# ShunyaoWang/quadruped_locomotion

Hardware: AMD Instinct MI355X
Metric: control-step QP solves/sec (18-DoF, 4-contact) at 1/2/4/8 MI355X (higher is better)
Workload: dtype f64

## Files before the change

### quadruped_locomotion_amd/csrc/force_qp_coop.hpp

```cpp
#pragma once

#include "coop_lanes.hpp"

#if defined(__FAST_MATH__) || (defined(__FINITE_MATH_ONLY__) && __FINITE_MATH_ONLY__)
#error "force_qp_coop.hpp needs IEEE inf / NaN semantics: do not build this translation unit with -ffast-math / -ffinite-math-only"
#endif

#ifndef QL_QP_BLOCK_STAMP
#define QL_QP_BLOCK_STAMP(slot) QL_BLOCK_STAMP(slot)
#endif
namespace qlamd {
namespace coop {

constexpr int kCoopLdsDoubles = 12 * 12;
constexpr int kMaxRefinePasses = 8;
#ifndef QLAMD_REFINE_AGAIN
#define QLAMD_REFINE_AGAIN 1e-3
#endif
constexpr double kRefineAgain = QLAMD_REFINE_AGAIN;
constexpr int kDropSlot = 48, kZeroSlot = 60, kWarmSlot = 61;
constexpr int kForceQpNrmRows = 5, kForceQpNrmRowsTorque = 8;
template <class T>
constexpr T one_v = T(1);
constexpr int kStatusWarmRejected = 6;
struct ForceQp {
  double Gm[12];
  double g0;
  double nb[3], t1[3], t2[3];
  double myn, myt1, myt2;
  double mu, f_min;
  bool on, comp;
  int nS;
  int refine_passes;
  double jrow[3], jcol[3];
  double tq_up, tq_lo;
  unsigned long long warm;
  unsigned stance;
  bool build_set;
};

__device__ __forceinline__ void force_qp_objective(const double S[6], double w_reg, double foot, unsigned stance, bool row_on,
                                                   const double F[6], const double *jrow, double w_tau_jt0, double Gm[12],
                                                   double &g0, double w_tau = 0.0) {
  const int lr = threadIdx.x & 15, leg = lr >> 2, c = lr & 3;
  const int myidx = 3 * leg + c;
  double r[4][3];
  static_for<12>([&](auto J) { constexpr int j = J; r[j / 3][j % 3] = bcv<j>(foot); });
  const double rl[3] = {quad_bc<0>(foot), quad_bc<1>(foot), quad_bc<2>(foot)};
  const double a[3] = {sel(c == 1, -rl[2], sel(c == 2, rl[1], 0.0)), sel(c == 0, rl[2], sel(c == 2, -rl[0], 0.0)),
                       sel(c == 0, -rl[1], sel(c == 1, rl[0], 0.0))};
  const double sa[3] = {S[3] * a[0], S[4] * a[1], S[5] * a[2]};
  const double Sfc = pick3(S, c);
#pragma unroll
  for (int m = 0; m < 4; m++) {
    const bool both = row_on && ((stance >> m) & 1u);
    const double xp = r[m][0], yp = r[m][1], zp = r[m][2];
    const double e0 = sa[1] * zp - sa[2] * yp;
    const double e1 = -sa[0] * zp + sa[2] * xp;
    const double e2 = sa[0] * yp - sa[1] * xp;
    Gm[3 * m + 0] = both ? e0 + (c == 0 ? Sfc : 0.0) : 0.0;
    Gm[3 * m + 1] = both ? e1 + (c == 1 ? Sfc : 0.0) : 0.0;
    Gm[3 * m + 2] = both ? e2 + (c == 2 ? Sfc : 0.0) : 0.0;
  }
  if (jrow) {
    double jj[3];
    static_for<3>([&](auto Bq) {
      constexpr int bq = Bq;
      jj[bq] = jrow[0] * quad_bc<bq>(jrow[0]) + jrow[1] * quad_bc<bq>(jrow[1]) + jrow[2] * quad_bc<bq>(jrow[2]);
    });
#pragma unroll
    for (int m = 0; m < 4; m++) {
      const bool own = row_on && m == leg;
#pragma unroll
      for (int bq = 0; bq < 3; bq++) Gm[3 * m + bq] += own ? w_tau * jj[bq] : 0.0;
    }
  }
#pragma unroll
  for (int j = 0; j < 12; j++)
    if (c < 3 && j == myidx) Gm[j] += row_on ? w_reg : 1.0;
  const double Fc = pick3(F, c);
  const double ST[3] = {S[3] * F[3], S[4] * F[4], S[5] * F[5]};
  const double g0v = -(Sfc * Fc + (a[0] * ST[0] + a[1] * ST[1] + a[2] * ST[2]) + w_tau_jt0);
  g0 = sel(row_on, g0v, 0.0);
}

template <bool kTorque, bool kWarm = false, int kLegs = 4, bool kRounds = true>
__device__ __forceinline__ int force_qp_coop(const ForceQp &Q, double *lds_row, double *lds_nrm, double &x, int &iters_out,
                                             unsigned long long *ws_out = nullptr) {
  using mask_t = std::conditional_t<kTorque, unsigned long long, unsigned>;
  constexpr int kKinds = kTorque ? 11 : 5;
  static_assert(kLegs == 2 || kLegs == 4, "legs in front of the row");
  constexpr int kV = 3 * kLegs;
  const int lr = threadIdx.x & 15, leg = lr >> 2, c = lr & 3;
  const bool comp = Q.comp && leg < kLegs, on = Q.on, row_on = comp && on;
  const int myidx = 3 * leg + c, nS = Q.nS;
  const double eps = 2.220446049250313e-16;
  const double inf = INFINITY;
  const double mu = Q.mu, f_min = Q.f_min, g0 = Q.g0;
  const double myn = Q.myn, myt1 = Q.myt1, myt2 = Q.myt2;
  const double *nb = Q.nb, *t1 = Q.t1, *t2 = Q.t2, *Gm = Q.Gm;
  double H[kV];
  double c1 = 0.0, c2 = 0.0;
  {
#pragma unroll
    for (int j = 0; j < kV; j++) H[j] = Gm[j];
    {
      double diag = 0.0;
#pragma unroll
      for (int j = 0; j < kV; j++) diag = (j == myidx) ? Gm[j] : diag;
      c1 = row_sum(sel(row_on, diag, 0.0));
    }
    bool bad = false;
    double my_pivot = 1.0;
    double d = bcv<0>(H[0]);
    static_for<kV>([&](auto K) {
      constexpr int k = K;
      bad = bad || !(d > 0.0);
      const double p = rcp_nr1(d);
      const bool piv = comp && (myidx == k);
      my_pivot = piv ? d : my_pivot;
      const double f = piv ? (1.0 - p) : H[k] * p;
      const double nf = -f;
      if constexpr (k < kV - 1) {
        fmac_bc<lane_of(k), true>(H[k + 1], H[k + 1], nf);
        d = bcv<k + 1>(H[k + 1]);
      }
      static_for<kV>([&](auto J) {
        constexpr int j = J;
        if constexpr (j != k && j != k + 1) fmac_bc<lane_of(k), (k == kV - 1 && j == 0)>(H[j], H[j], nf);
      });
      H[k] = piv ? p : nf;
    });
    const double rp = rsqrt_nr(my_pivot);
    c2 = row_sum(sel(row_on, rp, 0.0));
    if (bad && nS > 0) { iters_out = 0; return kStatusNotPd; }
  }

  QL_STAMP(5);
  x = 0.0;
  {
    const double ng0 = -g0;
    double xa[3] = {0.0, 0.0, 0.0};
    static_for<kV>([&](auto J) { constexpr int j = J; fmac_bc<lane_of(j), j == 0>(xa[j % 3], ng0, H[j]); });
    x = (xa[0] + xa[1]) + xa[2];
  }

  QL_STAMP(6); QL_QP_BLOCK_STAMP(6);
  double Ns[kV];
#pragma unroll
  for (int j = 0; j < kV; j++) Ns[j] = 0.0;
  double u = 0.0;
  int idk = 0;
  unsigned used = 0;
  int q = 0, iters = 0, status = kStatusOk;
  mask_t act_mask = 0, excl = 0;
  const double psi_tol = (double)(kKinds * nS) * eps * c1 * c2 * 100.0;
  double rnorm2 = 1.0;
  unsigned long long done_m = 0ull;
  int ip = 0;
  double sp = 0.0, ucand = 0.0, npj = 0.0;
  const double fa = c == 0 ? 1.0 : c == 1 ? -1.0 : 0.0, fb = c == 2 ? 1.0 : c == 3 ? -1.0 : 0.0;
  const double Wf0 = mu * nb[0] + (fa * t1[0] + fb * t2[0]), Wf1 = mu * nb[1] + (fa * t1[1] + fb * t2[1]),
               Wf2 = mu * nb[2] + (fa * t1[2] + fb * t2[2]);
  const mask_t one = 1;
  const mask_t maskf = on ? (one << (kKinds * leg + c + 1)) : 0, maskm = (on && c == 0) ? (one << (kKinds * leg)) : 0;
  const mask_t masku = (kTorque && on && comp) ? (one << (kKinds * leg + 5 + 2 * c)) : 0, maskl = masku << 1;
  constexpr int kTagBits = kTorque ? 2 : 1;
  constexpr unsigned kTagMask = (1u << (4 + kTagBits)) - 1u;
  const unsigned tagf = (unsigned)lr << kTagBits, tagm = tagf | 1u;
  const int row_addr = ((int)threadIdx.x & 48) << 2;
  const unsigned lanebit = 1u << lr;
  {
    const double nrm[5] = {myn, mu * myn + myt1, mu * myn - myt1, mu * myn + myt2, mu * myn - myt2};
#pragma unroll
    for (int k = 0; k < 5; k++) lds_nrm[64 * k + ((int)threadIdx.x & 63)] = nrm[k];
    lds_row[kZeroSlot] = 0.0;
    if constexpr (kTorque) {
#pragma unroll
      for (int k = 0; k < 3; k++) lds_nrm[64 * (5 + k) + ((int)threadIdx.x & 63)] = Q.jrow[k];
    }
  }
  const int nt_slot = comp ? kDropSlot + myidx : kZeroSlot;
  double zb = 0.0;
  double s_up = 0.0, s_lo = 0.0;
  const auto slacks = [&](double xx, double &s_min, double &s_fric) {
    const double x0 = quad_bc<0>(xx), x1 = quad_bc<1>(xx), x2 = quad_bc<2>(xx);
    s_fric = fma(Wf2, x2, fma(Wf1, x1, Wf0 * x0));
    s_min = fma(nb[2], x2, fma(nb[1], x1, fma(nb[0], x0, -f_min)));
    if constexpr (kTorque) {
      const double d = fma(Q.jcol[2], x2, fma(Q.jcol[1], x1, Q.jcol[0] * x0));
      s_up = Q.tq_up + d;
      s_lo = Q.tq_lo - d;
    }
  };
  const auto violation = [&](double s_min, double s_fric) -> double {
    double v = vmin(0.0, s_fric) + sel(c == 0, vmin(0.0, s_min), 0.0);
    if constexpr (kTorque) v += sel(comp, vmin(0.0, s_up) + vmin(0.0, s_lo), 0.0);
    return v;
  };
  const auto umax_dpp = [](unsigned k, auto Ctrl) -> unsigned {
    constexpr int ctrl = decltype(Ctrl)::value;
    const unsigned o = (unsigned)__builtin_amdgcn_mov_dpp((int)k, ctrl, 0xF, 0xF, true);
    return k > o ? k : o;
  };

  const auto latch = [&](bool newly) {
    if (newly) {
      lds_row[lr] = x;
      reinterpret_cast<int2 *>(lds_row + 16)[lr] = make_int2((int)used, idk);
      reinterpret_cast<int2 *>(lds_row + 32)[lr] = make_int2(q | (iters << 8), status);
      lds_row[nt_slot] = 0.0;
      lds_nrm[64 * 1 + ((int)threadIdx.x & 63)] = 0.0;
      zb = 0.0625; npj = 0.0;
    }
  };
  double vec = 0.0, hc = 0.0, nc = 0.0;
  const auto update_and_select = [&](auto Mode, bool resel, bool fresh, bool finished = false) -> bool {
    constexpr int kMode = decltype(Mode)::value;
    constexpr bool kUpd = kMode != 0;
    if constexpr (kMode == 1) {
      iters += (resel && fresh) ? 1 : 0;
      excl = (resel && fresh) ? 0 : excl;
    } else {
      iters += 1;
      excl = 0;
    }
    const mask_t avail = ~(act_mask | excl);
    double s_min, s_fric;
    slacks(x, s_min, s_fric);
    unsigned kf = __float_as_uint((float)s_fric), km = __float_as_uint((float)s_min);
    kf = ((avail & maskf) != 0 && s_fric < 0.0) ? ((kf & ~kTagMask) | tagf) : 0u;
    km = ((avail & maskm) != 0 && s_min < 0.0) ? ((km & ~kTagMask) | tagm) : 0u;
    double myv = km > kf ? s_min : s_fric;
    unsigned key = km > kf ? km : kf;
    if constexpr (kTorque) {
      const bool lower = s_lo < s_up;
      const double s_t = lower ? s_lo : s_up;
      unsigned kt = __float_as_uint((float)s_t);
      kt = ((avail & (lower ? maskl : masku)) != 0 && s_t < 0.0) ? ((kt & ~kTagMask) | tagf | (lower ? 3u : 2u)) : 0u;
      myv = kt > key ? s_t : myv;
      key = kt > key ? kt : key;
    }
    if constexpr (kUpd) {
      static_for<3>([&](auto J) { constexpr int j = J; fmac_bc<lane_of(j), j == 0>(H[j], vec, hc); fmac_bc<lane_of(j)>(Ns[j], vec, nc); });
    }
    key = umax_dpp(key, std::integral_constant<int, 0x128>{});
    if constexpr (kUpd) {
      static_for<3>([&](auto J) { constexpr int j = J + 3; fmac_bc<lane_of(j)>(H[j], vec, hc); fmac_bc<lane_of(j)>(Ns[j], vec, nc); });
    }
    key = umax_dpp(key, std::integral_constant<int, 0x124>{});
    if constexpr (kUpd) {
      static_for<2>([&](auto J) { constexpr int j = J + 6; if constexpr (j < kV) { fmac_bc<lane_of(j)>(H[j], vec, hc); fmac_bc<lane_of(j)>(Ns[j], vec, nc); } });
    }
    key = umax_dpp(key, std::integral_constant<int, 0x122>{});
    if constexpr (kUpd) {
      static_for<2>([&](auto J) { constexpr int j = J + 8; if constexpr (j < kV) { fmac_bc<lane_of(j)>(H[j], vec, hc); fmac_bc<lane_of(j)>(Ns[j], vec, nc); } });
    }
    key = umax_dpp(key, std::integral_constant<int, 0x121>{});
    const int wl = (int)(key >> kTagBits) & 15;
    const int addr = row_addr + (wl << 2);
    const int vlo = __builtin_amdgcn_ds_bpermute(addr, __double2loint(myv));
    const int vhi = __builtin_amdgcn_ds_bpermute(addr, __double2hiint(myv));
    int key_kind = (key & 1u) ? 0 : (wl & 3) + 1, tab_kind = key_kind;
    if constexpr (kTorque) {
      const bool tq = (key & 2u) != 0u;
      tab_kind = tq ? 5 + (wl & 3) : key_kind;
      key_kind = tq ? 5 + 2 * (wl & 3) + (int)(key & 1u) : key_kind;
    }
    const int key_ip = kKinds * (wl >> 2) + key_kind;
    double np_tab = lds_nrm[64 * tab_kind + ((int)threadIdx.x & 63)];
    if constexpr (kTorque) np_tab = ((key & 3u) == 3u) ? -np_tab : np_tab;
    if constexpr (kUpd) {
      static_for<2>([&](auto J) { constexpr int j = J + 10; if constexpr (j < kV) { fmac_bc<lane_of(j)>(H[j], vec, hc); fmac_bc<lane_of(j)>(Ns[j], vec, nc); } });
    }
    const double np_new = sel((wl >> 2) == leg, np_tab, 0.0);
    const bool any = (int)key < 0;
    const double v = __hiloint2double(vhi, vlo);
    bool feasible = false;
    const bool close = (kMode != 1 || (resel && fresh)) && any && !(v < -psi_tol);
    if (__builtin_amdgcn_ballot_w64(close) != 0ull) {
      const double psi = (double)row_sum_f32((float)sel(on, violation(s_min, s_fric), 0.0));
      feasible = close && (fabs(psi) <= psi_tol);
    }
    const bool stop = !any || feasible || iters > kMaxOuter;
    bool fin = stop;
    if constexpr (kMode == 1) {
      status = (resel && stop && iters > kMaxOuter) ? kStatusMaxIter : status;
      fin = (resel && stop) || finished;
      const bool take = resel && !stop;
      ip = take ? key_ip : ip;
      sp = sel(take, v, sp);
      ucand = sel(take, 0.0, ucand);
      npj = sel(take, np_new, npj);
    } else {
      status = (stop && iters > kMaxOuter) ? kStatusMaxIter : status;
      ip = key_ip; sp = v; ucand = 0.0; npj = np_new;
    }
    return fin;
  };
  const auto note_finished = [&](bool fin) {
    const unsigned long long fin_m = __builtin_amdgcn_ballot_w64(fin);
    const unsigned long long newly_m = fin_m & ~done_m;
    done_m |= fin_m;
    if (newly_m != 0ull) latch(__builtin_amdgcn_inverse_ballot_w64(newly_m));
  };
  const auto update_only = [&]() {
    static_for<kV>([&](auto J) {
      constexpr int j = J;
      fmac_bc<lane_of(j), j == 0>(H[j], vec, hc);
      fmac_bc<lane_of(j)>(Ns[j], vec, nc);
    });
  };
  double drop_einv = 0.0;
  const auto drop_vectors = [&](int lpos) {
    if (lr == lpos) {
#pragma unroll
      for (int j = 0; j < kV; j++) lds_row[kDropSlot + j] = Ns[j];
    }
    __builtin_amdgcn_fence(__ATOMIC_RELEASE, "wavefront");
    __builtin_amdgcn_s_waitcnt(0xC07F);
    const double nt_me = lds_row[nt_slot];
    const int drop_id = __shfl(idk, lpos, 16);
    double ga[3] = {0.0, 0.0, 0.0};
    static_for<kV>([&](auto J) { constexpr int j = J; fmac_bc<lane_of(j), j == 0>(ga[j % 3], nt_me, Gm[j]); });
    const double Gn = (ga[0] + ga[1]) + ga[2];
    const double einv = rcp_nr1(row_sum(fma(nt_me, Gn, zb)));
    drop_einv = einv;
    double ca[3] = {0.0, 0.0, 0.0};
    static_for<kV>([&](auto J) { constexpr int j = J; fmac_bc<lane_of(j), j == 0>(ca[j % 3], Gn, Ns[j]); });
    const double coef = (ca[0] + ca[1]) + ca[2];
    vec = nt_me;
    hc = nt_me * einv;
    nc = sel(lr == lpos, -1.0, -coef * einv);
    return drop_id;
  };

  int warm_updates = 0;
  QL_QP_BLOCK_STAMP(1);
  if constexpr (kWarm) {
    constexpr mask_t kLegRows = (one_v<mask_t> << kKinds) - 1;
    mask_t wm = (mask_t)Q.warm & (((Q.stance & 1u) ? kLegRows : 0) | ((Q.stance & 2u) ? kLegRows << kKinds : 0) |
                                  ((Q.stance & 4u) ? kLegRows << (2 * kKinds) : 0) | ((Q.stance & 8u) ? kLegRows << (3 * kKinds) : 0));
    {
      bool sane = true;
#pragma unroll
      for (int l = 0; l < 4; l++) {
        const mask_t rows = (wm >> (kKinds * l)) & kLegRows;
        int n = 0;
        if constexpr (kTorque) n = __popcll((unsigned long long)rows);
        else n = __popc((unsigned)rows);
        sane = sane && n <= 3;
      }
      wm = sane ? wm : (mask_t)0;
    }
#ifdef QLAMD_NO_GREEDY
    constexpr bool kGreedy = false;
#else
    constexpr bool kGreedy = kRounds;
#endif
    bool by_rounds = false, greedy = false;
    if constexpr (kRounds) {
      int nrows;
      if constexpr (kTorque) nrows = __popcll((unsigned long long)wm);
      else nrows = __popc((unsigned)wm);
      greedy = kGreedy && Q.build_set && wm == 0 && nS > 0;
      by_rounds = __builtin_amdgcn_ballot_w64(nrows >= (kLegs == 4 ? 6 : 4) || greedy) != 0ull;
    }
    if (by_rounds) {
      unsigned mine = (unsigned)((wm >> (kKinds * leg)) & kLegRows);
      const bool any_greedy = kGreedy && __builtin_amdgcn_ballot_w64(greedy) != 0ull;
      const auto rounds = [&](auto WithGreedy) {
      constexpr bool kWithGreedy = decltype(WithGreedy)::value;
      for (int round = 0;; round++) {
        bool have = mine != 0u;
        int kind = have ? __ffs((int)mine) - 1 : 0;
        mine &= mine - 1u;
        if constexpr (kWithGreedy) {
          if (round < 3) {
            double s_min, s_fric, xg = x;
            asm volatile("" : "+v"(xg));
            slacks(xg, s_min, s_fric);
            const mask_t avail = ~act_mask;
            unsigned kf = __float_as_uint((float)s_fric), km = __float_as_uint((float)s_min);
            kf = ((avail & maskf) != 0 && s_fric < 0.0) ? ((kf & ~kTagMask) | tagf) : 0u;
            km = ((avail & maskm) != 0 && s_min < 0.0) ? ((km & ~kTagMask) | tagm) : 0u;
            unsigned key = km > kf ? km : kf;
            if constexpr (kTorque) {
              const bool lower = s_lo < s_up;
              const double s_t = lower ? s_lo : s_up;
              unsigned kt = __float_as_uint((float)s_t);
              kt = ((avail & (lower ? maskl : masku)) != 0 && s_t < 0.0) ? ((kt & ~kTagMask) | tagf | (lower ? 3u : 2u)) : 0u;
              key = kt > key ? kt : key;
            }
            key = umax_dpp(key, std::integral_constant<int, 0xB1>{});
            key = umax_dpp(key, std::integral_constant<int, 0x4E>{});
            const bool ghave = greedy && (int)key < 0;
            const int cw = (int)((key >> kTagBits) & 3u);
            int gkind = (key & 1u) ? 0 : cw + 1;
            if constexpr (kTorque) gkind = (key & 2u) ? 5 + 2 * cw + (int)(key & 1u) : gkind;
            have = greedy ? ghave : have;
            kind = greedy ? gkind : kind;
          }
        }
        if (__builtin_amdgcn_ballot_w64(have) == 0ull) break;
        double nv, bp;
        {
          const double fr = sel(kind == 1, myt1, sel(kind == 2, -myt1, sel(kind == 3, myt2, -myt2)));
          nv = sel(kind == 0, myn, fma(mu, myn, fr));
          bp = sel(kind == 0, f_min, 0.0);
          if constexpr (kTorque) {
            const bool tq = kind >= 5, lower = tq && ((kind - 5) & 1) != 0;
            const int kj = (kind - 5) >> 1;
            const double jn = pick3(Q.jrow, kj);
            nv = sel(tq, sel(lower, -jn, jn), nv);
            const double bu = sel(kj == 0, quad_bc<0>(Q.tq_up), sel(kj == 1, quad_bc<1>(Q.tq_up), quad_bc<2>(Q.tq_up)));
            const double bl = sel(kj == 0, quad_bc<0>(Q.tq_lo), sel(kj == 1, quad_bc<1>(Q.tq_lo), quad_bc<2>(Q.tq_lo)));
            bp = sel(tq, -sel(lower, bl, bu), bp);
          }
        }
        npj = sel(have && comp, nv, 0.0);
        unsigned kinds = (have && c == 0) ? (unsigned)(kind + 1) << (4 * leg) : 0u;
        static_for<4>([&](auto K) {
          constexpr int ctrl = K == 0 ? 0x128 : K == 1 ? 0x124 : K == 2 ? 0x122 : 0x121;
          kinds |= (unsigned)__builtin_amdgcn_mov_dpp((int)kinds, ctrl, 0xF, 0xF, true);
        });
        double sl = quad_sum(npj * x) - sel(have, bp, 0.0);
        double za[kLegs], ra[kLegs];
#pragma unroll
        for (int m = 0; m < kLegs; m++) { za[m] = 0.0; ra[m] = 0.0; }
        static_for<kV>([&](auto J) {
          constexpr int j = J;
          fmac_bc<lane_of(j), j == 0>(za[j / 3], npj, H[j]);
          fmac_bc<lane_of(j)>(ra[j / 3], npj, Ns[j]);
        });
        static_for<kLegs>([&](auto K) {
          constexpr int k = K;
          const int kk = (int)((kinds >> (4 * k)) & 15u) - 1;
          const double qk = quad_sum(npj * za[k]);
          const double dk = bc<4 * k>(qk);
          const bool ok = kk >= 0 && dk > 1e-6;
          const double okf = sel(ok, 1.0, 0.0);
          const double zi = rcp_nr1(sel(ok, dk, 1.0)) * okf;
          const double zk = za[k] * okf, rr = ra[k] * okf;
          const double tw = -bc<4 * k>(sl) * zi;
          x = fma(tw, zk, x);
          u = fma(-tw, rr, u);
          sl = fma(tw, qk, sl);
          const int newlane = __ffs(~used & 0xFFFu) - 1;
          const bool newslot = ok && lr == newlane;
          const int pk = kKinds * k + kk;
          vec = zk * zi;
          hc = -zk;
          const double rk = sel(newslot, -1.0, rr);
          nc = -rk;
          u = sel(newslot, tw, u);
          idk = newslot ? pk : idk;
          used |= ok ? (1u << newlane) : 0u;
          act_mask |= ok ? (one << pk) : 0;
          rnorm2 = vmax(rnorm2, dk);
          q += ok ? 1 : 0;
          if constexpr (k + 1 < kLegs) {
            const double cm = -qk * zi;
            static_for<kLegs - 1 - k>([&](auto M) {
              constexpr int m = k + 1 + M;
              fmac_bc<4 * m, M == 0>(za[m], cm, zk);
              fmac_bc<4 * m>(ra[m], cm, rk);
            });
          }
          update_only();
        });
      }
      };
      if constexpr (kGreedy) {
        if (__builtin_expect(any_greedy, 0)) rounds(std::true_type{});
        else rounds(std::false_type{});
      } else {
        rounds(std::false_type{});
      }
    } else {
      for (;;) {
        const bool has = wm != 0;
        if (__builtin_amdgcn_ballot_w64(has) == 0ull) break;
        int p = 0;
        if constexpr (kTorque) p = has ? __ffsll((long long)wm) - 1 : 0;
        else p = has ? __ffs((int)wm) - 1 : 0;
        wm &= wm - 1;
        const int pleg = kTorque ? ((p * 47) >> 9) : id_leg(p), kind = p - kKinds * pleg;
        int tab_kind = kind;
        double sign = 1.0, b_p = sel(kind == 0, f_min, 0.0);
        if constexpr (kTorque) {
          const int kj = (kind - 5) >> 1;
          const bool tq = kind >= 5, lower = tq && ((kind - 5) & 1) != 0;
          tab_kind = tq ? 5 + kj : kind;
          sign = lower ? -1.0 : 1.0;
          const int src = 4 * pleg + (tq ? kj : 0);
          const double bu = __shfl(Q.tq_up, src, 16), bl = __shfl(Q.tq_lo, src, 16);
          b_p = tq ? -(lower ? bl : bu) : b_p;
        }
        const double np_tab = sign * lds_nrm[64 * tab_kind + ((int)threadIdx.x & 63)];
        npj = (has && pleg == leg) ? np_tab : 0.0;
        double za[3] = {0.0, 0.0, 0.0}, ra[3] = {0.0, 0.0, 0.0};
        static_for<kV>([&](auto J) {
          constexpr int j = J;
          fmac_bc<lane_of(j), j == 0>(za[j % 3], npj, H[j]);
          fmac_bc<lane_of(j)>(ra[j % 3], npj, Ns[j]);
        });
        const double zw = (za[0] + za[1]) + za[2], rw = (ra[0] + ra[1]) + ra[2];
        const double znw = row_sum(zw * npj);
        const double s_p = row_sum(npj * x) - b_p;
        const bool ok = has && znw > 1e-6;
        const double zi = rcp_nr(sel(ok, znw, 1.0));
        const double tw = sel(ok, -s_p * zi, 0.0);
        x = fma(tw, zw, x);
        u = fma(-tw, rw, u);
        const int newlane = __ffs(~used & 0xFFFu) - 1;
        const bool newslot = ok && lr == newlane;
        vec = sel(ok, zw * zi, 0.0);
        hc = sel(ok, -zw, 0.0);
        nc = sel(newslot, 1.0, sel(ok, -rw, 0.0));
        u = sel(newslot, tw, u);
        idk = newslot ? p : idk;
        used |= ok ? (1u << newlane) : 0u;
        act_mask |= ok ? (one << p) : 0;
        rnorm2 = sel(ok, vmax(rnorm2, znw), rnorm2);
        q += ok ? 1 : 0;
        warm_updates += ok ? 1 : 0;
        update_only();
      }
    }
    if (by_rounds) warm_updates = q;
    for (;;) {
      const bool slot = (used & lanebit) != 0u;
      const double umin = row_min(sel(slot, u, inf));
      const bool neg = umin < 0.0;
      if (__builtin_amdgcn_ballot_w64(neg) == 0ull) break;
      const int lpos = neg ? row_first(slot && u == umin) : 0;
      const double uk = __shfl(u, lpos, 16);
      const int drop_id = drop_vectors(lpos);
      x = sel(neg, fma(-hc, uk, x), x);
      u = sel(neg, fma(nc, uk, u), u);
      vec = sel(neg, vec, 0.0); hc = sel(neg, hc, 0.0); nc = sel(neg, nc, 0.0);
      act_mask &= neg ? ~(one << drop_id) : ~(mask_t)0;
      used &= neg ? ~(1u << lpos) : ~0u;
      q -= neg ? 1 : 0;
      warm_updates += neg ? 1 : 0;
      update_only();
    }
    npj = 0.0;
    if (lr == 0) reinterpret_cast<int *>(lds_row + kWarmSlot)[0] = warm_updates;
    warm_updates = 0;
  }
  QL_QP_BLOCK_STAMP(2);
  {
    done_m = ~__builtin_amdgcn_ballot_w64(true);
    const bool fin0 = update_and_select(std::integral_constant<int, 0>{}, true, true);
    note_finished(fin0);
  }

  double z = 0.0, r = 0.0, zn = 0.0, zinv = 0.0, t = 0.0, tl1 = 0.0, tl2 = 0.0, ratio = 0.0;
  const auto add_step = [&]() -> bool {
    x += t * z;
    u = fma(-t, r, u);
    const int newlane = __ffs(~used & 0xFFFu) - 1;
    const bool newslot = lr == newlane;
    vec = z * zinv;
    hc = -z;
    nc = sel(newslot, 1.0, -r);
    u = sel(newslot, ucand + t, u);
    idk = newslot ? ip : idk;
    used |= 1u << newlane;
    act_mask |= one << ip;
    rnorm2 = vmax(rnorm2, zn);
    q += 1;
    return update_and_select(std::integral_constant<int, 2>{}, true, true);
  };
  const auto drop_step = [&]() {
    const double tp = (tl2 >= inf) ? 0.0 : t;
    x += tp * z;
    u = fma(-t, r, u);
    ucand += t;
    sp += tp * zn;
    const int lpos = row_first(ratio == tl1 && ratio < inf);
    const double r_lpos = __shfl(r, lpos, 16);
    const int drop_id = drop_vectors(lpos);
    act_mask &= ~(one << drop_id);
    used &= ~(1u << lpos);
    q--;
    update_only();
    z = fma(hc, r_lpos, z);
    r = fma(nc, r_lpos, r);
    zn = fma(r_lpos * r_lpos, drop_einv, zn);
  };
  const auto general_dirs = [&]() {
    double za[3] = {0.0, 0.0, 0.0}, ra[3] = {0.0, 0.0, 0.0};
    static_for<kV>([&](auto J) {
      constexpr int j = J;
      fmac_bc<lane_of(j), j == 0>(za[j % 3], npj, H[j]);
      fmac_bc<lane_of(j)>(ra[j % 3], npj, Ns[j]);
    });
    z = (za[0] + za[1]) + za[2];
    r = (ra[0] + ra[1]) + ra[2];
    zn = row_sum(fma(z, npj, zb));
  };
  const auto step_lengths = [&]() -> bool {
    const bool slot = (used & lanebit) != 0u;
    const float zf = (float)z;
    const double zz = (double)row_sum_f32(zf * zf);
    const double ur = u * rcp_nr1(r);
    ratio = sel(slot && r > 0.0, ur, inf);
    tl1 = row_min(ratio);
    zinv = rcp_nr(zn);
    const double t2v = -sp * zinv;
    const bool exhausted = q >= 3 * nS;
    tl2 = sel((int)(!exhausted) & (int)(fabs(zz) > eps) & (int)(!(t2v < 0.0)), t2v, inf);
    t = vmin(tl1, tl2);
    return (tl2 < inf) && (tl2 <= tl1) && (zn > eps * eps * rnorm2);
  };
  const auto general_pass = [&](bool is_add) -> bool {
    const bool infeasible = !(t < inf);
    const bool dual_only = (tl2 >= inf);
    const bool full = !infeasible && !dual_only && (tl2 <= tl1);
    const bool degenerate = full && !is_add;
    const bool is_drop = !infeasible && !full;
    if (infeasible) status = kStatusInfeasible;
    const double tp = (infeasible || dual_only || degenerate) ? 0.0 : t;
    const double td = (infeasible || degenerate) ? 0.0 : t;
    x += tp * z;
    u = fma(-td, r, u);
    ucand += td;
    sp += tp * zn;
    const int newlane = __ffs(~used & 0xFFFu) - 1;
    const bool newslot = is_add && (lr == newlane);
    vec = is_add ? z * zinv : 0.0;
    hc = is_add ? -z : 0.0;
    nc = sel(newslot, 1.0, sel(is_add, -r, 0.0));
    u = newslot ? ucand : u;
    idk = newslot ? ip : idk;
    used |= is_add ? (1u << newlane) : 0u;
    act_mask |= is_add ? (one << ip) : 0;
    rnorm2 = is_add ? vmax(rnorm2, zn) : rnorm2;
    q += is_add ? 1 : 0;
    excl |= degenerate ? (one << ip) : 0;
    int lpos = 16;
    if (is_drop) {
      lpos = row_first(ratio == tl1 && ratio < inf);
      const int drop_id = drop_vectors(lpos);
      act_mask &= ~(one << drop_id);
      used &= ~(1u << lpos);
      q--;
    }
    return update_and_select(std::integral_constant<int, 1>{}, full, is_add, infeasible);
  };
  const auto in = [](unsigned long long m) -> bool { return __builtin_amdgcn_inverse_ballot_w64(m); };
  if (~done_m != 0ull) {
    for (;;) {
      unsigned long long add_m = 0ull;
      for (;;) {
        general_dirs();
        add_m = __builtin_amdgcn_ballot_w64(step_lengths());
        if (~(add_m | done_m) != 0ull) break;
        note_finished(add_step());
        if (~done_m == 0ull) break;
      }
      if (~done_m == 0ull) break;
      unsigned long long gen_m = 0ull;
      bool fin = false;
      for (;;) {
        const unsigned long long live_m = ~done_m & ~gen_m;
        const unsigned long long drop_m = __builtin_amdgcn_ballot_w64(tl1 < tl2) & live_m & ~add_m;
        const unsigned long long other_m = live_m & ~add_m & ~drop_m;
        if (other_m != 0ull) {
          if (in(other_m)) fin = general_pass(false);
          gen_m |= other_m;
        }
        if (drop_m == 0ull) break;
        if (in(drop_m | done_m)) drop_step();
        add_m = __builtin_amdgcn_ballot_w64(step_lengths());
      }
      const unsigned long long adders_m = add_m & ~done_m & ~gen_m;
      if (adders_m != 0ull) {
        bool fin_add = false;
        if (in(adders_m | done_m)) fin_add = add_step();
        fin = fin || (fin_add && in(adders_m));
      }
      note_finished(fin);
      if (~done_m == 0ull) break;
    }
  }
  {
    __builtin_amdgcn_fence(__ATOMIC_RELEASE, "wavefront");
    __builtin_amdgcn_s_waitcnt(0xC07F);
    x = lds_row[lr];
    const int2 a = reinterpret_cast<const int2 *>(lds_row + 16)[lr], b = reinterpret_cast<const int2 *>(lds_row + 32)[lr];
    used = (unsigned)a.x; idk = a.y; q = b.x & 255; status = b.y;
    if constexpr (kWarm) warm_updates = reinterpret_cast<const int *>(lds_row + kWarmSlot)[0];
    iters_out = (b.x >> 8) + warm_updates;
  }
  if constexpr (kWarm) {
    const mask_t mine = ((used >> lr) & 1u) ? (one_v<mask_t> << idk) : 0;
    unsigned lo = (unsigned)mine, hi = 0u;
    if constexpr (kTorque) hi = (unsigned)((unsigned long long)mine >> 32);
    static_for<4>([&](auto K) {
      constexpr int ctrl = K == 0 ? 0x128 : K == 1 ? 0x124 : K == 2 ? 0x122 : 0x121;
      lo |= (unsigned)__builtin_amdgcn_mov_dpp((int)lo, ctrl, 0xF, 0xF, true);
      if constexpr (kTorque) hi |= (unsigned)__builtin_amdgcn_mov_dpp((int)hi, ctrl, 0xF, 0xF, true);
    });
    if (ws_out) *ws_out = status == kStatusOk ? ((unsigned long long)hi << 32 | lo) : 0ull;
  }

  QL_STAMP(7); QL_QP_BLOCK_STAMP(7);
  if (status == kStatusOk && (q > 0 || (kWarm && warm_updates > 0))) {
    if (lr < kV) {
#pragma unroll
      for (int j = 0; j < kV; j++) lds_row[12 * lr + j] = Ns[j];
    }
    __builtin_amdgcn_fence(__ATOMIC_RELEASE, "wavefront");
    __builtin_amdgcn_s_waitcnt(0xC07F);
    double NsT[kV];
#pragma unroll
    for (int k = 0; k < kV; k++) NsT[k] = comp ? lds_row[12 * k + myidx] : 0.0;
    const int lg = kTorque ? ((idk * 47) >> 9) : id_leg(idk), tt = idk - kKinds * lg;
    const bool myslot = (used >> lr) & 1u;
    const int src = myslot ? (4 * lg + (tt == 0 ? 0 : (tt < 5 ? tt - 1 : (tt - 5) >> 1))) : 0;
    int passes = Q.refine_passes;
    if constexpr (kWarm) passes += warm_updates > 0 ? iters_out >> 4 : 0;
    for (int pass = 0; pass < passes; pass++) {
      double grad = g0;
      static_for<kV>([&](auto J) { constexpr int j = J; fmac_bc<lane_of(j), j == 0>(grad, x, Gm[j]); });
      double corr = 0.0;
      static_for<kV>([&](auto J) { constexpr int j = J; fmac_bc<lane_of(j), j == 0>(corr, grad, H[j]); });
      x -= corr;
      double s_min, s_fric;
      slacks(x, s_min, s_fric);
      const double vm = __shfl(s_min, src, 16), vf = __shfl(s_fric, src, 16);
      double res = sel(tt == 0, vm, vf);
      if constexpr (kTorque) {
        const double vu = __shfl(s_up, src, 16), vl = __shfl(s_lo, src, 16);
        res = sel(tt < 5, res, sel(((tt - 5) & 1) != 0, vl, vu));
      }
      const double rho = sel(myslot, -res, 0.0);
      double dx = 0.0;
      static_for<kV>([&](auto K) { constexpr int k = K; fmac_bc<k, k == 0>(dx, rho, NsT[k]); });
      x += dx;
      if constexpr (kWarm) {
        const double moved = -row_min(-(__builtin_fabs(corr) + __builtin_fabs(dx)));
        passes += (warm_updates > 0 && pass + 1 == passes && passes < kMaxRefinePasses && moved > kRefineAgain) ? 1 : 0;
      }
    }
  }

  if constexpr (kWarm) {
    if (__builtin_amdgcn_ballot_w64(status == kStatusOk && warm_updates > 0) != 0ull) {
      double s_min, s_fric;
      slacks(x, s_min, s_fric);
      double worst = vmin(s_fric, sel(c == 0, s_min, s_fric));
      if constexpr (kTorque) worst = sel(comp, vmin(worst, vmin(s_up, s_lo)), worst);
      const double wmin = row_min(sel(on, worst, 0.0));
      double grad = g0;
      static_for<kV>([&](auto J) { constexpr int j = J; fmac_bc<lane_of(j), j == 0>(grad, x, Gm[j]); });
      double ua[3] = {0.0, 0.0, 0.0};
      static_for<kV>([&](auto J) { constexpr int j = J; fmac_bc<lane_of(j), j == 0>(ua[j % 3], grad, Ns[j]); });
      const bool myslot2 = ((used >> lr) & 1u) != 0u;
      const double umin = row_min(sel(myslot2, (ua[0] + ua[1]) + ua[2], 0.0));
      const bool accept = wmin > -1e-6 && umin > -1e-6;
      status = (status == kStatusOk && warm_updates > 0 && !accept) ? kStatusWarmRejected : status;
    }
  }
  return status;
}

}
}
```

Baseline: 297.2 million.

## Batch per-leg rank-one active-set updates via small Cholesky-style elimination

For the non-torque QP path, the per-leg sequential rank-one updates are restructured. The code now computes all leg cross products (quad_sum reductions) up front into a small 4x4 Gram matrix and performs an LDL-like elimination in registers. The H and Ns updates are then applied afterward in one batched pass, replacing interleaved reduction/broadcast per leg. This cuts dependent cross-lane reductions in exchange for more register use and different floating-point rounding order.

```diff
diff --git a/quadruped_locomotion_amd/csrc/force_qp_coop.hpp b/quadruped_locomotion_amd/csrc/force_qp_coop.hpp
--- a/quadruped_locomotion_amd/csrc/force_qp_coop.hpp
+++ b/quadruped_locomotion_amd/csrc/force_qp_coop.hpp
@@ -433,6 +433,67 @@
           fmac_bc<lane_of(j), j == 0>(za[j / 3], npj, H[j]);
           fmac_bc<lane_of(j)>(ra[j / 3], npj, Ns[j]);
         });
+        if constexpr (!kTorque) {
+          double qs[kLegs];
+          static_for<kLegs>([&](auto K) { constexpr int k = K; qs[k] = quad_sum(npj * za[k]); });
+          double D[kLegs][kLegs];
+          double sk[kLegs];
+          static_for<kLegs>([&](auto K) {
+            constexpr int k = K;
+            static_for<k + 1>([&](auto M) { constexpr int m = M; D[m][k] = bc<4 * m>(qs[k]); });
+            sk[k] = bc<4 * k>(sl);
+          });
+          double W[kLegs][kLegs], L[kLegs][kLegs], zi[kLegs], tw[kLegs];
+          static_for<kLegs>([&](auto K) {
+            constexpr int k = K;
+            const int kk = (int)((kinds >> (4 * k)) & 15u) - 1;
+            double dk = D[k][k], s = sk[k];
+            static_for<k>([&](auto J) {
+              constexpr int j = J;
+              dk = fma(-L[k][j], W[k][j], dk);
+              s = fma(tw[j], W[k][j], s);
+            });
+            const bool ok = kk >= 0 && dk > 1e-6;
+            const double okf = sel(ok, 1.0, 0.0);
+            zi[k] = rcp_nr1(sel(ok, dk, 1.0)) * okf;
+            tw[k] = -s * zi[k];
+            static_for<kLegs - 1 - k>([&](auto Mq) {
+              constexpr int m = k + 1 + Mq;
+              double w = D[k][m];
+              static_for<k>([&](auto J) { constexpr int j = J; w = fma(-L[k][j], W[m][j], w); });
+              W[m][k] = w;
+              L[m][k] = w * zi[k];
+            });
+            static_for<k>([&](auto J) {
+              constexpr int j = J;
+              za[k] = fma(-L[k][j], za[j], za[k]);
+              ra[k] = fma(-L[k][j], ra[j], ra[k]);
+            });
+            za[k] *= okf;
+            const double rr = ra[k] * okf;
+            x = fma(tw[k], za[k], x);
+            u = fma(-tw[k], rr, u);
+            const int newlane = __ffs(~used & 0xFFFu) - 1;
+            const bool newslot = ok && lr == newlane;
+            const int pk = kKinds * k + kk;
+            ra[k] = sel(newslot, -1.0, rr);
+            u = sel(newslot, tw[k], u);
+            idk = newslot ? pk : idk;
+            used |= ok ? (1u << newlane) : 0u;
+            act_mask |= ok ? (one << pk) : 0;
+            rnorm2 = vmax(rnorm2, dk);
+            q += ok ? 1 : 0;
+          });
+          static_for<kLegs>([&](auto K) {
+            constexpr int k = K;
+            const double nvk = za[k] * -zi[k];
+            static_for<kV>([&](auto J) {
+              constexpr int j = J;
+              fmac_bc<lane_of(j), j == 0>(H[j], nvk, za[k]);
+              fmac_bc<lane_of(j)>(Ns[j], nvk, ra[k]);
+            });
+          });
+        } else
         static_for<kLegs>([&](auto K) {
           constexpr int k = K;
           const int kk = (int)((kinds >> (4 * k)) & 15u) - 1;
```

New measurement: 304.5 million, median of 6. 1.02x the previous value.
